# rimelq/VISTAF-RoboSkin-Vision-Integrated-Multimodal-Sensor

Hardware: AMD Instinct MI355X
Metric: frames/sec (224x224 -> force-map) at batch 256 (higher is better)
Workload: dtype f32; 1 GPU; BASELINE configs[2]: batch 256/GPU of 224x224x3 fp16 fringe frames (256 distinct frames) -> 224x224 f32 depth map + force scalars, full FTP path (inpaint, demod, unwrap, detrend, compose, force tail), constants scaled-224; inputs resident in HBM; global_batch=256, input_dtype=fp16, constants=scaled, parallelism=dp1, inflight_batches=3, frames_with_nonzero_status=0

## Files before the change

vistaf-roboskin-vision-integrated-multimodal-sensor_amd/_lib.py:

```python
from __future__ import annotations

import ctypes
import os

_HERE = os.path.dirname(os.path.abspath(__file__))
LIB_PATH = os.path.join(_HERE, "libvistaf_ftp.so")

NSCALARS = 16
NREFINFO = 8
NCONTACT = 16
MAX_CONTACTS = 64
NTRACK = 16
TRACK_NAMES = ["track_id", "age_frames", "parent_row", "events", "overlap_px", "dx", "dy", "dforce_N", "dvolume_cm3", "origin_track_id"]
TRACK_EVENTS = {"born": 1, "split": 2, "merged": 4, "gated": 8}
FATE_ENDED, FATE_NO_ROW = -1, -2 ** 31
NSHAPE = 24
SHAPE_NAMES = ["contact_pixels", "boundary_pixels", "footprint_cx", "footprint_cy", "major_axis_mm", "minor_axis_mm", "orientation_rad",
               "fit_pixels", "fit_status", "apex_x", "apex_y", "apex_depth_mm", "curvature_1_per_mm", "curvature_2_per_mm",
               "curvature_axis_rad", "radius_1_mm", "radius_2_mm", "fit_rms_mm"]
SHAPE_FIT = {"ok": 0, "none": 1, "not_a_cap": 2}
NTAXEL, NTAXELFRAME, TAXEL_NONE = 12, 8, 0xFFFF
TAXEL_NAMES = ["contact_pixels", "contact_area_mm2", "volume_cm3", "mean_depth_mm", "max_depth_mm", "argmax_index", "centroid_x", "centroid_y",
               "force_N", "pressure_kPa"]
TAXEL_FRAME_NAMES = ["active_taxels", "volume_cm3", "force_N", "cop_x", "cop_y", "moment_x_Nmm", "moment_y_Nmm", "peak_taxel"]
# ... 223 lines not shown
        "vistaf_motion_reset": (ci, [vp]),
        "vistaf_motion_destroy": (None, [vp]),
    },
    "PRESSURE_EXPORTS": {
        "vistaf_pressure_create": (ci, [ci, ci, ci, ci, ci, cd, cd, cd, P(vp)]),
        "vistaf_pressure_measure": (ci, [vp, vp, vp, vp, vp, vp, vp, vp, cf, ci, vp, vp, vp, vp]),
        "vistaf_pressure_destroy": (None, [vp]),
    },
}
MASK_CHAIN_SIGNATURES = {
    "vistaf_ftp_test_mask_chain_fits": (ci, [ci, ci, ci, ci, ci, ci]),
    "vistaf_ftp_test_bad_chain": (ci, [vp, vp, vp, vp, vp, ci, ci, vp, vp, ci, ci, ci, ci, vp]),
    "vistaf_ftp_test_reliable_chain": (ci, [vp, vp, vp, ci, ci, ci, vp, vp, vp, vp, ci, ci, ci, ci, vp]),
    "vistaf_ftp_test_contact_chain": (ci, [vp, vp, vp, vp, cd, cd, ci, ci, vp, vp, vp, vp, ci, ci, ci, ci, vp]),
}
OUTLINE_SIGNATURES = {
    "vistaf_outline_workspace_bytes": (ci, [ci, ci, ci, ci, P(sz)]),
    "vistaf_outline_measure": (ci, [vp, vp, vp, vp, ci, ci, ci, ci, ci, vp, vp, vp, vp, sz, vp]),
}
TEXTURE_SIGNATURES = {
    "vistaf_texture_workspace_bytes": (ci, [ci, ci, ci, ci, ci, P(sz)]),
    "vistaf_texture_measure": (ci, [vp, vp, vp, vp, vp, cf, cd, ci, ci, cd, cd, ci, ci, ci, ci, vp, vp, vp, vp, sz, vp]),
}
MATCH_SIGNATURES = {
    "vistaf_match_bank_bytes": (ci, [ci, ci, ci, P(i32), P(sz)]),
    "vistaf_match_build_bank": (ci, [P(cf), P(i32), P(i32), ci, ci, ci, cd, vp, sz]),
    "vistaf_match_workspace_bytes": (ci, [ci, ci, ci, ci, ci, ci, ci, P(sz)]),
    "vistaf_match_measure": (ci, [vp, vp, vp, vp, vp, vp, sz, P(i32), cf, ci, ci, cd, cd, ci, ci, ci, ci, vp, vp, vp, vp, sz, vp]),
}
(EXPORTS, ALIGN_EXPORTS, TEST_EXPORTS, TEMP_EXPORTS, TEMPMODEL_EXPORTS, TSENSOR_EXPORTS, TRACK_EXPORTS, SHAPE_EXPORTS, TAXEL_EXPORTS, THERMAL_EXPORTS,
 TEMPORAL_EXPORTS, CLOUD_EXPORTS, MOTION_EXPORTS, PRESSURE_EXPORTS) = (list(group) for group in SIGNATURES.values())

_lib = None


def load():
    global _lib
    if _lib is not None:
        return _lib
    if not os.path.exists(LIB_PATH):
        raise RuntimeError(
            f"{LIB_PATH} is missing: build it with `python __graft_entry__.py` (hipcc --offload-arch=gfx950). "
            "This package has no CPU path."
        )
    lib = ctypes.CDLL(LIB_PATH)
    for group in list(SIGNATURES.values()) + [MASK_CHAIN_SIGNATURES, OUTLINE_SIGNATURES, TEXTURE_SIGNATURES, MATCH_SIGNATURES]:
        for name, (restype, argtypes) in group.items():
            fn = getattr(lib, name)
            fn.restype, fn.argtypes = restype, argtypes
    _lib = lib
    return lib


def check(rc: int):
    if rc != 0:
        msg = load().vistaf_ftp_last_error().decode("utf-8", "replace")
        if rc == -1:
            raise ValueError(msg)
        raise RuntimeError(f"vistaf_ftp error {rc}: {msg}")
```

vistaf-roboskin-vision-integrated-multimodal-sensor_amd/csrc/api.hip:

```cpp
#include <hip/hip_runtime.h>
#include <algorithm>
#include <cmath>
#include <cstdio>
#include <cstdlib>
#include <cstring>
#include <map>
#include <string>
#include <vector>

#include "host_util.hpp"
#include "mask_rules.hpp"
#include "mask_bits.hpp"

using namespace vf;
#include "test_hooks.h"
#include "test_hooks_masks.h"
#ifdef VISTAF_DEBUG
namespace vf { void telea_debug_dump(); void telea_window_debug_dump(int B); void telea_window_mw_debug_dump(int B); void fit_debug_dump(); void unwrap_big_debug_dump(); void unwrap_batch_debug_dump(); }
#endif

static thread_local std::string g_err;
static int fail(int code, const std::string &msg) { g_err = msg; return code; }
namespace vf { int set_error(int code, const std::string &msg) { return fail(code, msg); } }

namespace {

struct GKern { float *d = nullptr; int k = 0; };

enum Stage { ST_GRAY_BAD = 0, ST_INPAINT, ST_PREPROC, ST_DEMOD, ST_RELIABLE, ST_UNWRAP_RANK, ST_UNWRAP, ST_UNWRAP_TREE, ST_DETREND, ST_SMOOTH_FLIP, ST_COMPOSE, ST_MM_BLOB,
             ST_TAIL, ST_COUNT };
const char *kStageNames[ST_COUNT] = {"gray+badpix", "inpaint (k_telea_window_mw)", "illum+blur+apod+median", "pruned-dft demod", "reliable mask",
// ... 512 lines not shown
    preprocess(hd, d_ref, format, 1, st, false);
    int rc = reference_search(hd, 1, hd->geom, st);
    if (rc) return rc;
    CarrierGeom g;
    HIPCHK(hipMemcpyAsync(&g, hd->geom, sizeof(g), hipMemcpyDeviceToHost, st));
    HIPCHK(hipStreamSynchronize(st));
    if (!g.ok) return fail(VISTAF_E_NOCARRIER, "no carrier peak in the reference spectrum");
    hd->peak_x = g.peak_x; hd->peak_y = g.peak_y; hd->kx = g.kx; hd->ky = g.ky;
    hd->ph = g.ph; hd->pw = g.pw;
    {
        std::vector<float> win = hann_patch(g.ph, g.pw);
        HIPCHK(hipMemcpyAsync(hd->win, win.data(), win.size() * sizeof(float), hipMemcpyHostToDevice, st));
        HIPCHK(hipStreamSynchronize(st));
    }
    launch_build_tables(hd->geom, 0, hd->Ex, hd->Ey, hd->Gx, hd->Gy, 0, 0, 1, h, w, pad, Hf, Wf, hd->pmax, st);
    launch_dft_forward(hd->iw, hd->mu, hd->Ex, hd->Ey, 0, 0, hd->win, hd->tmpT, hd->patch, hd->pmax * hd->pmax, 1, h, w, hd->ph, hd->pw, st);
    launch_dft_inverse(hd->patch, hd->pmax * hd->pmax, hd->Gx, hd->Gy, 0, 0, hd->tmpT, hd->cref, hd->amp_ref, nullptr, nullptr, 0, nullptr, nullptr,
                       1, h, w, hd->ph, hd->pw, st);
    HIPCHK(hipStreamSynchronize(st));
    hd->period = g.period;
    hd->mm_per_px = hd->period > 1e-12 ? c.grating_pitch_mm / hd->period : 0.0;
    hd->have_ref = true;
    return 0;
}

int vistaf_ftp_get_reference_info(const vistaf_ftp_handle *hd, double *o)
{
    if (!hd || !o) return fail(VISTAF_E_INVALID, "null argument");
    if (!hd->have_ref) return fail(VISTAF_E_STATE, "set_reference has not been called");
    o[0] = hd->peak_x; o[1] = hd->peak_y; o[2] = hd->kx; o[3] = hd->ky; o[4] = hd->Hf; o[5] = hd->Wf; o[6] = hd->period; o[7] = hd->mm_per_px;
    return 0;
}

// ... 130 lines not shown
{
    if (!hd || !d_frames) return fail(VISTAF_E_INVALID, "null argument");
    if (!hd->have_ref) return fail(VISTAF_E_STATE, "set_reference has not been called");
    if (B < 1 || B > hd->maxB) return fail(VISTAF_E_STATE, "batch exceeds max_batch");
    TRY(check_frames(hd, format, d_frames, nullptr));
    if (!(hd->period > 1e-12)) return fail(VISTAF_E_STATE, "Invalid estimated_grating_period_px");
    hipStream_t st = (hipStream_t)stream;
    int h = hd->h, w = hd->w;
    bool timed = hd->timing;
    if (timed) ensure_events(hd);
    HIPCHK(hipMemsetAsync(hd->status, 0, sizeof(int32_t) * B, st));

    preprocess(hd, d_frames, format, B, st, timed);

    if (timed) hipEventRecord(hd->ev[ST_DEMOD], st);
    launch_dft_forward(hd->iw, hd->mu, hd->Ex, hd->Ey, 0, 0, hd->win, hd->tmpT, hd->patch, hd->pmax * hd->pmax, B, h, w, hd->ph, hd->pw, st);
    launch_dft_inverse(hd->patch, hd->pmax * hd->pmax, hd->Gx, hd->Gy, 0, 0, hd->tmpT, hd->keep_planes ? hd->field : nullptr, hd->amp, hd->cref,
                       hd->amp_ref, 0, hd->prod, hd->wrapped, B, h, w, hd->ph, hd->pw, st);
    return post_demod(hd, B, d_height_mm, d_reliable, d_scalars, d_status, nullptr, st);
}

int vistaf_ftp_predict_pairs(vistaf_ftp_handle *hd, const void *d_refs, const void *d_defs, int format, int B, float *d_height_mm,
                             uint8_t *d_reliable, double *d_scalars, int32_t *d_status, void *stream)
{
    if (!hd || !d_refs || !d_defs) return fail(VISTAF_E_INVALID, "null argument");
    if (B < 1 || B > hd->maxB) return fail(VISTAF_E_STATE, "batch exceeds max_batch");
    TRY(check_frames(hd, format, d_refs, d_defs));
    hipStream_t st = (hipStream_t)stream;
    const vistaf_ftp_config &c = hd->cfg;
    int h = hd->h, w = hd->w, P = hd->P, pad = std::max(0, c.fft_pad_px), pm = hd->pmax;
    bool timed = hd->timing;
    if (timed) ensure_events(hd);
    if (!hd->pairs_ready) {
// ... 13 lines not shown
    }
    HIPCHK(hipMemsetAsync(hd->status, 0, sizeof(int32_t) * B, st));
    const size_t sx = (size_t)w * pm, sy = (size_t)h * pm;
    const bool together = 2 * B <= hd->maxB;
    const float *iw_def = hd->iw, *mu_def = hd->mu;
    const int *bad_def = hd->bad_count;
    if (together) {
        HIPCHK(hipMemsetAsync(hd->status + B, 0, sizeof(int32_t) * B, st));
        preprocess(hd, d_refs, format, B, st, timed, d_defs);
        iw_def = hd->iw + (size_t)B * P; mu_def = hd->mu + B; bad_def = hd->bad_count + B;
    } else preprocess(hd, d_refs, format, B, st, false);
    int rc = reference_search(hd, B, hd->pgeom, st);
    if (rc) return rc;
    launch_pair_status(hd->pgeom, pm, hd->status, together ? hd->status + B : nullptr, B, st);
    launch_build_tables(hd->pgeom, 1, hd->pEx, hd->pEy, hd->pGx, hd->pGy, sx, sy, B, h, w, pad, hd->Hf, hd->Wf, pm, st, hd->hann_tab, hd->pwin);
    launch_dft_forward(hd->iw, hd->mu, hd->pEx, hd->pEy, sx, sy, hd->pwin, hd->tmpT, hd->patch, pm * pm, B, h, w, pm, pm, st, pm * pm);
    launch_dft_inverse(hd->patch, pm * pm, hd->pGx, hd->pGy, sx, sy, hd->tmpT, hd->pcref, hd->pamp_ref, nullptr, nullptr, 0, nullptr, nullptr, B, h, w,
                       pm, pm, st, hd->pgeom);
    if (!together) preprocess(hd, d_defs, format, B, st, timed);
    if (timed) hipEventRecord(hd->ev[ST_DEMOD], st);
    launch_dft_forward(iw_def, mu_def, hd->pEx, hd->pEy, sx, sy, hd->pwin, hd->tmpT, hd->patch, pm * pm, B, h, w, pm, pm, st, pm * pm);
    launch_dft_inverse(hd->patch, pm * pm, hd->pGx, hd->pGy, sx, sy, hd->tmpT, hd->keep_planes ? hd->field : nullptr, hd->amp, hd->pcref, hd->pamp_ref,
                       (size_t)P, hd->prod, hd->wrapped, B, h, w, pm, pm, st, hd->pgeom);
    return post_demod(hd, B, d_height_mm, d_reliable, d_scalars, d_status, hd->pgeom, st, bad_def);
}

int vistaf_ftp_get_pair_info(vistaf_ftp_handle *hd, int batch, double *out , void *stream)
{
    if (!hd || !out) return fail(VISTAF_E_INVALID, "null argument");
    if (!hd->pairs_ready || batch < 1 || batch > hd->maxB) return fail(VISTAF_E_STATE, "predict_pairs has not been called");
    std::vector<CarrierGeom> g(batch);
    HIPCHK(hipMemcpyAsync(g.data(), hd->pgeom, sizeof(CarrierGeom) * batch, hipMemcpyDeviceToHost, (hipStream_t)stream));
    HIPCHK(hipStreamSynchronize((hipStream_t)stream));
    for (int b = 0; b < batch; b++) {
        double *o = out + (size_t)b * VISTAF_NREFINFO;
        o[0] = g[b].peak_x; o[1] = g[b].peak_y; o[2] = g[b].kx; o[3] = g[b].ky; o[4] = hd->Hf; o[5] = hd->Wf; o[6] = g[b].period;
        o[7] = g[b].period > 1e-12 ? hd->cfg.grating_pitch_mm / g[b].period : 0.0;
    }
// ... 41 lines not shown
int vistaf_ftp_test_set(vistaf_ftp_handle *hd, const char *name, int value)
{
    if (!hd || !name) return fail(VISTAF_E_INVALID, "null argument");
    const std::string n(name);
    if (n == "inpaint_tier" && value >= 0 && value <= 2) hd->tiers.inpaint = value;
    else if (n == "big_flood_handback") hd->tiers.big_flood_handback = value != 0;
    else if (n == "chamfer_twopass") hd->tiers.chamfer_twopass = value != 0;
    else if (n == "telea_two_tier") hd->tiers.telea_two_tier = value != 0;
    else if (n == "telea_mw") hd->tiers.telea_mw = value != 0;
    else if (n == "big_queue_lds") hd->tiers.big_queue_lds = value != 0;
    else if (n == "big_gq_cap" && (value == 0 || (value >= 64 && (value & (value - 1)) == 0))) hd->tiers.big_gq_cap = value;
    else if (n == "big_fallback") hd->tiers.big_fallback = value != 0;
    else if (n == "unwrap_fast") hd->tiers.unwrap_fast = value != 0;
    else if (n == "big_chain") hd->tiers.big_chain = value != 0;
    else if (n == "select_resident") hd->tiers.select_resident = value != 0;
    else if (n == "fused_chains") hd->tiers.fused_chains = value != 0;
    else if (n == "fused_backend") hd->tiers.fused_backend = value != 0;
    else if (n == "fused_masks" && value >= 0 && value <= 7) hd->tiers.fused_masks = value;
    else if (n == "keep_planes") hd->keep_planes = value != 0;
    else return fail(VISTAF_E_INVALID, "unknown test hook or value: " + n);
    return 0;
}

namespace {
int hook_scratch(int variant, int B, int h, int w, bool chain_ok, void **scratch)
{
    *scratch = nullptr;
    if (variant < 0 || variant > 2) return fail(VISTAF_E_INVALID, "variant must be 0, 1 or 2");
    if (variant == 2 && !chain_ok) return fail(VISTAF_E_INVALID, "variant 2: the k_big.hip chain does not take this batch");
    if (variant == 1 || (variant == 0 && !large_frame((size_t)h * w))) return 0;
// ... 405 lines not shown
        (void)hipFree(geom); (void)hipFree(hann);
        return fail(VISTAF_E_HIP, "memcpy geometry");
    }
    launch_build_tables(geom, geom_stride, (double2 *)Ex, (double2 *)Ey, (double2 *)Gx, (double2 *)Gy, (size_t)w * pmax, (size_t)h * pmax, B, h, w, pad, Hf,
                        Wf, pmax, st, pair ? hann : nullptr, pair ? win : nullptr);
    return hook_finish(geom, hann, st);
}

int vistaf_ftp_test_build_full_tables(void *Exf, void *Eyf, int h, int w, int pad, int Hf, int Wf, void *stream)
{
    if (!Exf || !Eyf || !dft_sizes_ok(1, h, w) || !padded_ok(h, w, pad, Hf, Wf)) return fail(VISTAF_E_INVALID, "bad argument");
    launch_build_full_tables((double2 *)Exf, (double2 *)Eyf, h, w, pad, Hf, Wf, (hipStream_t)stream);
    return hook_finish(nullptr, nullptr, (hipStream_t)stream);
}

int vistaf_ftp_test_dft_forward(const float *iw, const float *mu, const void *Ex, const void *Ey, size_t tab_stride_x, size_t tab_stride_y, const float *win,
                                int win_stride, void *T, void *patch, int patch_stride, int B, int h, int w, int ph, int pw, void *stream)
{
    if (!iw || !Ex || !Ey || !win || !T || !patch || !dft_sizes_ok(B, h, w) || ph < 1 || pw < 1 || ph > 4096 || pw > 4096 ||
        (size_t)B * h * pw > 0x7fffffffull)
        return fail(VISTAF_E_INVALID, "bad argument");
    if ((tab_stride_x == 0) != (tab_stride_y == 0) || (tab_stride_x && (tab_stride_x < (size_t)w * pw || tab_stride_y < (size_t)ph * h)) ||
        (win_stride != 0 && win_stride < ph * pw) || patch_stride < ph * pw)
        return fail(VISTAF_E_INVALID, "a stride is smaller than what it strides over, or only one table stride is zero");
    launch_dft_forward(iw, mu, (const double2 *)Ex, (const double2 *)Ey, tab_stride_x, tab_stride_y, win, (double2 *)T, (double2 *)patch, patch_stride, B, h, w,
                       ph, pw, (hipStream_t)stream, win_stride);
    return hook_finish(nullptr, nullptr, (hipStream_t)stream);
}

int vistaf_ftp_test_dft_inverse(const void *patch, int patch_stride, const void *Gx, const void *Gy, size_t tab_stride_x, size_t tab_stride_y, void *Q, void *field,
                                float *amp, const void *cref, const float *amp_ref, size_t ref_stride, float *prod, float *wrapped, const int32_t *gi_or_null,
                                int B, int h, int w, int ph, int pw, void *stream)
{
    if (!patch || !Gx || !Gy || !Q || !amp || (cref && (!amp_ref || !prod || !wrapped)) || !dft_sizes_ok(B, h, w) || ph < 1 || pw < 1 || ph > 4096 ||
        pw > 4096 || (size_t)B * ph * w > 0x7fffffffull)
        return fail(VISTAF_E_INVALID, "bad argument");
    if ((tab_stride_x == 0) != (tab_stride_y == 0) || (tab_stride_x && (tab_stride_x < (size_t)w * pw || tab_stride_y < (size_t)ph * h)) ||
        patch_stride < ph * pw || (ref_stride != 0 && ref_stride < (size_t)h * w))
        return fail(VISTAF_E_INVALID, "a stride is smaller than what it strides over, or only one table stride is zero");
    hipStream_t st = (hipStream_t)stream;
    CarrierGeom *geom = nullptr;
    if (gi_or_null) {
        const double zeros[7] = {0, 0, 0, 0, 0, 0, 0};
        std::vector<CarrierGeom> g((size_t)B);
        for (int b = 0; b < B; b++) g[b] = geom_pack(zeros, gi_or_null + 10 * (size_t)b);
        HIPCHK(hipMalloc((void **)&geom, g.size() * sizeof(CarrierGeom)));
        if (hipMemcpy(geom, g.data(), g.size() * sizeof(CarrierGeom), hipMemcpyHostToDevice) != hipSuccess) {
            (void)hipFree(geom);
            return fail(VISTAF_E_HIP, "memcpy geometry");
        }
    }
    launch_dft_inverse((const double2 *)patch, patch_stride, (const double2 *)Gx, (const double2 *)Gy, tab_stride_x, tab_stride_y, (double2 *)Q, (double2 *)field, amp,
                       (const double2 *)cref, amp_ref, ref_stride, prod, wrapped, B, h, w, ph, pw, st, geom);
    return hook_finish(geom, nullptr, st);
}

int vistaf_depth_map_to_volume(const float *d_height, const uint8_t *d_roi, int batch, int h, int w, double mm_per_px,
                               double depth_eps_mm, double *d_out, void *stream)
{
    if (!d_height || !d_out || batch < 1 || h < 1 || w < 1) return fail(VISTAF_E_INVALID, "bad argument");
    PostParams pp;
    pp.mm_per_px = mm_per_px; pp.depth_eps_mm = depth_eps_mm; pp.period_px = 0; pp.force_curve = Curve{0, 0, 0, 0};
    launch_tail(d_height, d_roi, nullptr, nullptr, pp, nullptr, 0, d_out, batch, h * w, (hipStream_t)stream);
    return launch_ok("launch");
}

int vistaf_predict_force_from_volume(const vistaf_curve *curve, double volume_cm3, double *force_out)
{
// ... 9 lines not shown
```

vistaf-roboskin-vision-integrated-multimodal-sensor_amd/csrc/cgemm_mfma.hpp:

```cpp
#pragma once
#include <hip/hip_runtime.h>

namespace vf {

typedef double v4f64 __attribute__((ext_vector_type(4)));

__device__ __forceinline__ void cgemm16x64_mfma(const double *__restrict__ A, int lda, int kext, const double2 *__restrict__ Q, int ldq, int ncols,
                                                int ya, int x0, int lane, v4f64 (&cre)[4], v4f64 (&cim)[4])
{
    const int r = lane & 15, kk = lane >> 4;
#pragma unroll
    for (int t = 0; t < 4; t++) { cre[t] = (v4f64){0.0, 0.0, 0.0, 0.0}; cim[t] = (v4f64){0.0, 0.0, 0.0, 0.0}; }
    const int K = 2 * kext;
    for (int k0 = 0; k0 < K; k0 += 4) {
        const int k = k0 + kk;
        const bool in = k < K, hi = k >= kext;
        const int kq = in ? (hi ? k - kext : k) : 0;
        const double a = in ? A[((size_t)ya * lda + kq) * 2 + (hi ? 1 : 0)] : 0.0;
        double2 q[4];
#pragma unroll
        for (int t = 0; t < 4; t++) q[t] = Q[(size_t)kq * ldq + min(x0 + 16 * t + r, ncols - 1)];
#pragma unroll
        for (int t = 0; t < 4; t++) {
            const double bre = in ? (hi ? -q[t].y : q[t].x) : 0.0, bim = in ? (hi ? q[t].x : q[t].y) : 0.0;
            cre[t] = __builtin_amdgcn_mfma_f64_16x16x4f64(a, bre, cre[t], 0, 0, 0);
            cim[t] = __builtin_amdgcn_mfma_f64_16x16x4f64(a, bim, cim[t], 0, 0, 0);
        }
    }
}

}
```

vistaf-roboskin-vision-integrated-multimodal-sensor_amd/csrc/k_dft.hip:

```cpp
#include <algorithm>
#include "kernels.hpp"
#include "cgemm_mfma.hpp"

namespace vf {

__device__ inline void cmac(double &ar, double &ai, double er, double ei, double vr, double vi)
{
    ar = fma(er, vr, ar); ar = fma(-ei, vi, ar);
    ai = fma(er, vi, ai); ai = fma(ei, vr, ai);
}

constexpr int DFT_MAXT = 4;
__global__ __launch_bounds__(256) void k_dft_fwd1_mfma(const float *__restrict__ iw, const float *__restrict__ mu, const double2 *__restrict__ Ex_all,
                                                       size_t ex_stride, double2 *__restrict__ T, int h, int w, int pw, int seg_rows, int nseg)
{
    const int lane = threadIdx.x & 63, wid = threadIdx.x >> 6;
    const int sps = (seg_rows + 15) / 16;
    const int strip = blockIdx.x * 4 + wid;
    if (strip >= nseg * sps) return;
    const int seg = strip / sps;
    const int row0 = seg * seg_rows + (strip - seg * sps) * 16;
    const int row_end = (seg + 1) * seg_rows;
    const int r = lane & 15, kk = lane >> 4;
    const int grow = min(row0 + r, row_end - 1);
// ... 22 lines not shown
                if (t0 + t < ntile) acc[t] = __builtin_amdgcn_mfma_f64_16x16x4f64(a, bv[t], acc[t], 0, 0, 0);
        }
#pragma unroll
        for (int t = 0; t < DFT_MAXT; t++) {
            if (eoff[t] < 0) continue;
            const int n = (t0 + t) * 16 + r, c = n < pw ? n : n - pw;
#pragma unroll
            for (int q = 0; q < 4; q++) {
                const int row = row0 + kk + 4 * q;
                if (row < row_end) ((double *)(T + (size_t)row * pw + c))[n < pw ? 0 : 1] = acc[t][q];
            }
        }
    }
}

__global__ void k_dft_fwd2(const double2 *__restrict__ T, const double2 *__restrict__ Ey_all, size_t ey_stride, const float *__restrict__ win_all,
                           int win_stride, double2 *__restrict__ patch, int h, int ph, int pw, int pstride)
{
    size_t b = blockIdx.x;
    const double2 *Ey = Ey_all + b * ey_stride;
    const float *win = win_all + b * (size_t)win_stride;
    const double2 *Tb = T + b * (size_t)h * pw;
    for (int t = threadIdx.x; t < ph * pw; t += blockDim.x) {
        int a = t / pw, c = t % pw;
        double ar = 0.0, ai = 0.0;
        int y = 0;
        for (; y + 8 <= h; y += 8) {
            double2 e[8], v[8];
#pragma unroll
            for (int k = 0; k < 8; k++) { e[k] = Ey[(size_t)a * h + y + k]; v[k] = Tb[(size_t)(y + k) * pw + c]; }
#pragma unroll
            for (int k = 0; k < 8; k++) cmac(ar, ai, e[k].x, e[k].y, v[k].x, v[k].y);
        }
        for (; y < h; y++) {
            const double2 e = Ey[(size_t)a * h + y], v = Tb[(size_t)y * pw + c];
            cmac(ar, ai, e.x, e.y, v.x, v.y);
        }
        const double wv = (double)win[t];
        patch[b * (size_t)pstride + t] = make_double2(ar * wv, ai * wv);
    }
}

void launch_dft_forward(const float *iw, const float *mu, const double2 *Ex, const double2 *Ey, size_t tab_stride_x, size_t tab_stride_y,
                        const float *win, double2 *tmpT, double2 *patch, int patch_stride, int B, int h, int w, int ph, int pw, hipStream_t st,
                        int win_stride)
{
    const int seg_rows = tab_stride_x ? h : B * h, nseg = tab_stride_x ? B : 1;
    const int strips = nseg * ((seg_rows + 15) / 16);
    hipLaunchKernelGGL(k_dft_fwd1_mfma, dim3((strips + 3) / 4), dim3(256), 0, st, iw, mu, Ex, tab_stride_x, tmpT, h, w, pw, seg_rows, nseg);
    hipLaunchKernelGGL(k_dft_fwd2, dim3(B), dim3(std::min(1024, ((ph * pw + 63) / 64) * 64)), 0, st, (const double2 *)tmpT, Ey, tab_stride_y, win, win_stride, patch, h,
                       ph, pw, patch_stride);
}

__global__ void k_dft_inv1(const double2 *__restrict__ patch, int pstride, const double2 *__restrict__ Gx_all, size_t gx_stride,
                           double2 *__restrict__ Q, int w, int ph, int pw, const CarrierGeom *__restrict__ geom)
{
    int x = blockIdx.x * blockDim.x + threadIdx.x;
    int a = blockIdx.y;
    size_t b = blockIdx.z;
    if (x >= w) return;
    const int pwb = geom ? max(0, min(geom[b].pw, pw)) : pw;
    if (geom && a >= max(0, min(geom[b].ph, ph))) return;
    const double2 *Gx = Gx_all + b * gx_stride;
    const double2 *pr = patch + b * (size_t)pstride + (size_t)a * pw;
// ... 35 lines not shown
            const size_t p = (size_t)y * w + x, i = b * (size_t)h * w + p;
            if (field) field[i] = make_double2(ar, ai);
            const float am = (float)sqrt(fma(ar, ar, ai * ai));
            amp[i] = am;
            if (cref) {
                const double2 c = cref[p];
                const double rr = ar * c.x + ai * c.y;
                const double ri = ai * c.x - ar * c.y;
                wrapped[i] = (float)atan2(ri, rr);
                prod[i] = __fmul_rn(amp_ref[p], am);
            }
        }
    }
}

void launch_dft_inverse(const double2 *patch, int patch_stride, const double2 *Gx, const double2 *Gy, size_t tab_stride_x, size_t tab_stride_y,
                        double2 *tmpQ, double2 *field, float *amp, const double2 *cref, const float *amp_ref, size_t ref_stride, float *prod,
                        float *wrapped, int B, int h, int w, int ph, int pw, hipStream_t st, const CarrierGeom *geom)
{
    hipLaunchKernelGGL(k_dft_inv1, dim3((w + 255) / 256, ph, B), dim3(256), 0, st, patch, patch_stride, Gx, tab_stride_x, tmpQ, w, ph, pw, geom);
    hipLaunchKernelGGL(k_dft_inv2_mfma, dim3((w + 63) / 64, (h + 63) / 64, B), dim3(256), 0, st, (const double2 *)tmpQ, Gy, tab_stride_y, field, amp, cref,
                       amp_ref, ref_stride, prod, wrapped, h, w, ph, geom);
}

__global__ __launch_bounds__(256) void k_full2_mfma(const double2 *__restrict__ T, const double2 *__restrict__ Eyf, double *__restrict__ mag_all,
                                                    int h, int Hf, int Wf, int Wh)
{
    const int lane = threadIdx.x & 63, wid = threadIdx.x >> 6;
    const int x0 = blockIdx.x * 64, y0 = (blockIdx.y * 4 + wid) * 16;
    const size_t b = blockIdx.z;
    if (y0 >= Hf) return;
    const int r = lane & 15, kk = lane >> 4;
    const double *G = (const double *)Eyf;
    const double2 *Tb = T + b * (size_t)h * Wh;
    const int ya = min(y0 + r, Hf - 1);
    v4f64 cre[4], cim[4];
    cgemm16x64_mfma(G, h, h, Tb, Wh, Wh, ya, x0, lane, cre, cim);
// ... 147 lines not shown
```

vistaf-roboskin-vision-integrated-multimodal-sensor_amd/csrc/kernels.hpp:

```cpp
#pragma once
#include <hip/hip_runtime.h>
#include <stdint.h>
#include <vector>
#include "common.hpp"

namespace vf {

struct Tiers {
    int inpaint = 2;
    int big_flood_handback = 0;
    int chamfer_twopass = 0;
    int telea_two_tier = 1;
    int unwrap_fast = 1;
    int big_chain = 1;
    int big_queue_lds = 1;
    int big_gq_cap = 0;
    int big_fallback = 1;
    int telea_mw = 1;
    int fused_backend = 1;
    int select_resident = 1;
    int fused_masks = 7;
    int fused_chains = 1;
};

inline bool large_frame(size_t P) { return P >= 262144; }

struct ScratchLayout;
struct ScratchRegion;
using ScratchRec = std::vector<ScratchRegion>;

struct RowSpanSE {
    int k;
    int8_t lo[33];
    int8_t hi[33];
};

// ... 35 lines not shown
                          float *const *outs, int *counts, int B, int P, hipStream_t st);

struct CarrierGeom {
    double peak_x, peak_y;
    double kx, ky;
    double dpx, dpy;
    double period;
    int x0, y0, ph, pw;
    int px_i, py_i;
    int px_raw, py_raw;
    int ok;
    int keep_carrier;
};
void launch_dft_forward(const float *iw, const float *mu, const double2 *Ex, const double2 *Ey, size_t tab_stride_x, size_t tab_stride_y,
                        const float *win, double2 *tmpT, double2 *patch, int patch_stride, int B, int h, int w, int ph, int pw, hipStream_t st,
                        int win_stride = 0);
void launch_dft_inverse(const double2 *patch, int patch_stride, const double2 *Gx, const double2 *Gy, size_t tab_stride_x, size_t tab_stride_y,
                        double2 *tmpQ, double2 *field, float *amp, const double2 *cref, const float *amp_ref, size_t ref_stride, float *prod,
                        float *wrapped, int B, int h, int w, int ph, int pw, hipStream_t st, const CarrierGeom *geom = nullptr);
void launch_dft_full_mag(const float *iw, const float *mu, const double2 *Ex_full, const double2 *Ey_full, double2 *tmp,
                         double *mag, int B, int h, int w, int Hf, int Wf, hipStream_t st);
void launch_dft_rows(const float *iw, const float *mu, const double2 *Ex, double2 *T, int B, int h, int w, int nc, hipStream_t st);
void launch_top_peaks(const double *mag, int B, int Hf, int Wf, int dc, int npeaks, double *out_xyv , hipStream_t st);
void launch_carrier_choose(const double *peaks, int npk, const double *mag, int Hf, int Wf, int bw, double max_dy_frac, CarrierGeom *geom, int B,
                           hipStream_t st);
void launch_build_tables(const CarrierGeom *geom, int geom_stride, double2 *Ex, double2 *Ey, double2 *Gx, double2 *Gy, size_t stride_x,
                         size_t stride_y, int B, int h, int w, int pad, int Hf, int Wf, int pmax, hipStream_t st, const float *pair_hann = nullptr,
                         float *pair_win = nullptr);
void launch_pair_status(const CarrierGeom *geom, int pmax, int32_t *status, const int32_t *status2, int B, hipStream_t st);
void launch_build_full_tables(double2 *Exf, double2 *Eyf, int h, int w, int pad, int Hf, int Wf, hipStream_t st);

void launch_threshold_mask(const float *q, const uint8_t *roi, const float *thr, uint8_t *out, int B, int P, hipStream_t st);
enum CcLabelTier { CCT_LDS_MASK = 0, CCT_LDS = 1, CCT_GLOBAL = 2 };
int cc_label_tier(int h, int w, bool force_global = false);
// ... 161 lines not shown
```

Before: 75890 frames/s.

## Add LDS-staged MFMA kernels for forward row DFT and inverse column DFT

Measured after the change: 76690 frames/s, median of 6. 1.01x the previous value.

```diff
diff --git a/vistaf-roboskin-vision-integrated-multimodal-sensor_amd/_lib.py b/vistaf-roboskin-vision-integrated-multimodal-sensor_amd/_lib.py
--- a/vistaf-roboskin-vision-integrated-multimodal-sensor_amd/_lib.py
+++ b/vistaf-roboskin-vision-integrated-multimodal-sensor_amd/_lib.py
@@ -261,6 +261,11 @@
     "vistaf_ftp_test_reliable_chain": (ci, [vp, vp, vp, ci, ci, ci, vp, vp, vp, vp, ci, ci, ci, ci, vp]),
     "vistaf_ftp_test_contact_chain": (ci, [vp, vp, vp, vp, cd, cd, ci, ci, vp, vp, vp, vp, ci, ci, ci, ci, vp]),
 }
+DFT_STAGED_SIGNATURES = {
+    "vistaf_ftp_test_dft_forward_v": (ci, [vp, vp, vp, vp, sz, sz, vp, ci, vp, vp, ci, ci, ci, ci, ci, ci, ci, vp]),
+    "vistaf_ftp_test_dft_inverse_v": (ci, [vp, ci, vp, vp, sz, sz, vp, vp, vp, vp, vp, sz, vp, vp, vp, ci, ci, ci, ci, ci, ci, vp]),
+    "vistaf_ftp_test_dft_staged_fits": (ci, [ci, ci, ci, ci, ci]),
+}
 OUTLINE_SIGNATURES = {
     "vistaf_outline_workspace_bytes": (ci, [ci, ci, ci, ci, P(sz)]),
     "vistaf_outline_measure": (ci, [vp, vp, vp, vp, ci, ci, ci, ci, ci, vp, vp, vp, vp, sz, vp]),
@@ -291,7 +296,7 @@
             "This package has no CPU path."
         )
     lib = ctypes.CDLL(LIB_PATH)
-    for group in list(SIGNATURES.values()) + [MASK_CHAIN_SIGNATURES, OUTLINE_SIGNATURES, TEXTURE_SIGNATURES, MATCH_SIGNATURES]:
+    for group in list(SIGNATURES.values()) + [MASK_CHAIN_SIGNATURES, DFT_STAGED_SIGNATURES, OUTLINE_SIGNATURES, TEXTURE_SIGNATURES, MATCH_SIGNATURES]:
         for name, (restype, argtypes) in group.items():
             fn = getattr(lib, name)
             fn.restype, fn.argtypes = restype, argtypes
diff --git a/vistaf-roboskin-vision-integrated-multimodal-sensor_amd/csrc/api.hip b/vistaf-roboskin-vision-integrated-multimodal-sensor_amd/csrc/api.hip
--- a/vistaf-roboskin-vision-integrated-multimodal-sensor_amd/csrc/api.hip
+++ b/vistaf-roboskin-vision-integrated-multimodal-sensor_amd/csrc/api.hip
@@ -15,6 +15,7 @@
 using namespace vf;
 #include "test_hooks.h"
 #include "test_hooks_masks.h"
+#include "test_hooks_dft.h"
 #ifdef VISTAF_DEBUG
 namespace vf { void telea_debug_dump(); void telea_window_debug_dump(int B); void telea_window_mw_debug_dump(int B); void fit_debug_dump(); void unwrap_big_debug_dump(); void unwrap_batch_debug_dump(); }
 #endif
@@ -557,9 +558,9 @@
         HIPCHK(hipStreamSynchronize(st));
     }
     launch_build_tables(hd->geom, 0, hd->Ex, hd->Ey, hd->Gx, hd->Gy, 0, 0, 1, h, w, pad, Hf, Wf, hd->pmax, st);
-    launch_dft_forward(hd->iw, hd->mu, hd->Ex, hd->Ey, 0, 0, hd->win, hd->tmpT, hd->patch, hd->pmax * hd->pmax, 1, h, w, hd->ph, hd->pw, st);
+    launch_dft_forward(hd->iw, hd->mu, hd->Ex, hd->Ey, 0, 0, hd->win, hd->tmpT, hd->patch, hd->pmax * hd->pmax, 1, h, w, hd->ph, hd->pw, st, 0, hd->tiers.dft_staged != 0);
     launch_dft_inverse(hd->patch, hd->pmax * hd->pmax, hd->Gx, hd->Gy, 0, 0, hd->tmpT, hd->cref, hd->amp_ref, nullptr, nullptr, 0, nullptr, nullptr,
-                       1, h, w, hd->ph, hd->pw, st);
+                       1, h, w, hd->ph, hd->pw, st, nullptr, hd->tiers.dft_staged != 0);
     HIPCHK(hipStreamSynchronize(st));
     hd->period = g.period;
     hd->mm_per_px = hd->period > 1e-12 ? c.grating_pitch_mm / hd->period : 0.0;
@@ -720,9 +721,9 @@
     preprocess(hd, d_frames, format, B, st, timed);
 
     if (timed) hipEventRecord(hd->ev[ST_DEMOD], st);
-    launch_dft_forward(hd->iw, hd->mu, hd->Ex, hd->Ey, 0, 0, hd->win, hd->tmpT, hd->patch, hd->pmax * hd->pmax, B, h, w, hd->ph, hd->pw, st);
+    launch_dft_forward(hd->iw, hd->mu, hd->Ex, hd->Ey, 0, 0, hd->win, hd->tmpT, hd->patch, hd->pmax * hd->pmax, B, h, w, hd->ph, hd->pw, st, 0, hd->tiers.dft_staged != 0);
     launch_dft_inverse(hd->patch, hd->pmax * hd->pmax, hd->Gx, hd->Gy, 0, 0, hd->tmpT, hd->keep_planes ? hd->field : nullptr, hd->amp, hd->cref,
-                       hd->amp_ref, 0, hd->prod, hd->wrapped, B, h, w, hd->ph, hd->pw, st);
+                       hd->amp_ref, 0, hd->prod, hd->wrapped, B, h, w, hd->ph, hd->pw, st, nullptr, hd->tiers.dft_staged != 0);
     return post_demod(hd, B, d_height_mm, d_reliable, d_scalars, d_status, nullptr, st);
 }
 
@@ -766,14 +767,14 @@
     if (rc) return rc;
     launch_pair_status(hd->pgeom, pm, hd->status, together ? hd->status + B : nullptr, B, st);
     launch_build_tables(hd->pgeom, 1, hd->pEx, hd->pEy, hd->pGx, hd->pGy, sx, sy, B, h, w, pad, hd->Hf, hd->Wf, pm, st, hd->hann_tab, hd->pwin);
-    launch_dft_forward(hd->iw, hd->mu, hd->pEx, hd->pEy, sx, sy, hd->pwin, hd->tmpT, hd->patch, pm * pm, B, h, w, pm, pm, st, pm * pm);
+    launch_dft_forward(hd->iw, hd->mu, hd->pEx, hd->pEy, sx, sy, hd->pwin, hd->tmpT, hd->patch, pm * pm, B, h, w, pm, pm, st, pm * pm, hd->tiers.dft_staged != 0);
     launch_dft_inverse(hd->patch, pm * pm, hd->pGx, hd->pGy, sx, sy, hd->tmpT, hd->pcref, hd->pamp_ref, nullptr, nullptr, 0, nullptr, nullptr, B, h, w,
-                       pm, pm, st, hd->pgeom);
+                       pm, pm, st, hd->pgeom, hd->tiers.dft_staged != 0);
     if (!together) preprocess(hd, d_defs, format, B, st, timed);
     if (timed) hipEventRecord(hd->ev[ST_DEMOD], st);
-    launch_dft_forward(iw_def, mu_def, hd->pEx, hd->pEy, sx, sy, hd->pwin, hd->tmpT, hd->patch, pm * pm, B, h, w, pm, pm, st, pm * pm);
+    launch_dft_forward(iw_def, mu_def, hd->pEx, hd->pEy, sx, sy, hd->pwin, hd->tmpT, hd->patch, pm * pm, B, h, w, pm, pm, st, pm * pm, hd->tiers.dft_staged != 0);
     launch_dft_inverse(hd->patch, pm * pm, hd->pGx, hd->pGy, sx, sy, hd->tmpT, hd->keep_planes ? hd->field : nullptr, hd->amp, hd->pcref, hd->pamp_ref,
-                       (size_t)P, hd->prod, hd->wrapped, B, h, w, pm, pm, st, hd->pgeom);
+                       (size_t)P, hd->prod, hd->wrapped, B, h, w, pm, pm, st, hd->pgeom, hd->tiers.dft_staged != 0);
     return post_demod(hd, B, d_height_mm, d_reliable, d_scalars, d_status, hd->pgeom, st, bad_def);
 }
 
@@ -845,6 +846,7 @@
     else if (n == "unwrap_fast") hd->tiers.unwrap_fast = value != 0;
     else if (n == "big_chain") hd->tiers.big_chain = value != 0;
     else if (n == "select_resident") hd->tiers.select_resident = value != 0;
+    else if (n == "dft_staged") hd->tiers.dft_staged = value != 0;
     else if (n == "fused_chains") hd->tiers.fused_chains = value != 0;
     else if (n == "fused_backend") hd->tiers.fused_backend = value != 0;
     else if (n == "fused_masks" && value >= 0 && value <= 7) hd->tiers.fused_masks = value;
@@ -1280,8 +1282,24 @@
     return hook_finish(nullptr, nullptr, (hipStream_t)stream);
 }
 
+namespace {
+int dft_hook_variant(int variant, int bit, int h, int w, int ph, int pw, bool per_frame, bool *staged)
+{
+    if (variant < 0 || variant > 2) return fail(VISTAF_E_INVALID, "variant must be 0, 1 or 2");
+    if (variant == 2 && !(dft_staged_fits(h, w, ph, pw, per_frame) & bit)) return fail(VISTAF_E_INVALID, "variant 2: the staged kernel does not take this shape");
+    *staged = variant != 1;
+    return 0;
+}
+}
+
 int vistaf_ftp_test_dft_forward(const float *iw, const float *mu, const void *Ex, const void *Ey, size_t tab_stride_x, size_t tab_stride_y, const float *win,
                                 int win_stride, void *T, void *patch, int patch_stride, int B, int h, int w, int ph, int pw, void *stream)
+{
+    return vistaf_ftp_test_dft_forward_v(iw, mu, Ex, Ey, tab_stride_x, tab_stride_y, win, win_stride, T, patch, patch_stride, B, h, w, ph, pw, 0, stream);
+}
+
+int vistaf_ftp_test_dft_forward_v(const float *iw, const float *mu, const void *Ex, const void *Ey, size_t tab_stride_x, size_t tab_stride_y, const float *win,
+                                  int win_stride, void *T, void *patch, int patch_stride, int B, int h, int w, int ph, int pw, int variant, void *stream)
 {
     if (!iw || !Ex || !Ey || !win || !T || !patch || !dft_sizes_ok(B, h, w) || ph < 1 || pw < 1 || ph > 4096 || pw > 4096 ||
         (size_t)B * h * pw > 0x7fffffffull)
@@ -1289,8 +1307,10 @@
     if ((tab_stride_x == 0) != (tab_stride_y == 0) || (tab_stride_x && (tab_stride_x < (size_t)w * pw || tab_stride_y < (size_t)ph * h)) ||
         (win_stride != 0 && win_stride < ph * pw) || patch_stride < ph * pw)
         return fail(VISTAF_E_INVALID, "a stride is smaller than what it strides over, or only one table stride is zero");
+    bool staged;
+    if (int rc = dft_hook_variant(variant, DFT_STAGED_FWD1, h, w, ph, pw, tab_stride_x != 0, &staged)) return rc;
     launch_dft_forward(iw, mu, (const double2 *)Ex, (const double2 *)Ey, tab_stride_x, tab_stride_y, win, (double2 *)T, (double2 *)patch, patch_stride, B, h, w,
-                       ph, pw, (hipStream_t)stream, win_stride);
+                       ph, pw, (hipStream_t)stream, win_stride, staged);
     return hook_finish(nullptr, nullptr, (hipStream_t)stream);
 }
 
@@ -1298,12 +1318,28 @@
                                 float *amp, const void *cref, const float *amp_ref, size_t ref_stride, float *prod, float *wrapped, const int32_t *gi_or_null,
                                 int B, int h, int w, int ph, int pw, void *stream)
 {
+    return vistaf_ftp_test_dft_inverse_v(patch, patch_stride, Gx, Gy, tab_stride_x, tab_stride_y, Q, field, amp, cref, amp_ref, ref_stride, prod, wrapped,
+                                         gi_or_null, B, h, w, ph, pw, 0, stream);
+}
+
+int vistaf_ftp_test_dft_staged_fits(int h, int w, int ph, int pw, int per_frame_tables)
+{
+    if (h < 1 || w < 1 || ph < 1 || pw < 1) return fail(VISTAF_E_INVALID, "bad argument");
+    return dft_staged_fits(h, w, ph, pw, per_frame_tables != 0);
+}
+
+int vistaf_ftp_test_dft_inverse_v(const void *patch, int patch_stride, const void *Gx, const void *Gy, size_t tab_stride_x, size_t tab_stride_y, void *Q,
+                                  void *field, float *amp, const void *cref, const float *amp_ref, size_t ref_stride, float *prod, float *wrapped,
+                                  const int32_t *gi_or_null, int B, int h, int w, int ph, int pw, int variant, void *stream)
+{
     if (!patch || !Gx || !Gy || !Q || !amp || (cref && (!amp_ref || !prod || !wrapped)) || !dft_sizes_ok(B, h, w) || ph < 1 || pw < 1 || ph > 4096 ||
         pw > 4096 || (size_t)B * ph * w > 0x7fffffffull)
         return fail(VISTAF_E_INVALID, "bad argument");
     if ((tab_stride_x == 0) != (tab_stride_y == 0) || (tab_stride_x && (tab_stride_x < (size_t)w * pw || tab_stride_y < (size_t)ph * h)) ||
         patch_stride < ph * pw || (ref_stride != 0 && ref_stride < (size_t)h * w))
         return fail(VISTAF_E_INVALID, "a stride is smaller than what it strides over, or only one table stride is zero");
+    bool staged;
+    if (int rc = dft_hook_variant(variant, DFT_STAGED_INV2, h, w, ph, pw, tab_stride_x != 0, &staged)) return rc;
     hipStream_t st = (hipStream_t)stream;
     CarrierGeom *geom = nullptr;
     if (gi_or_null) {
@@ -1317,7 +1353,7 @@
         }
     }
     launch_dft_inverse((const double2 *)patch, patch_stride, (const double2 *)Gx, (const double2 *)Gy, tab_stride_x, tab_stride_y, (double2 *)Q, (double2 *)field, amp,
-                       (const double2 *)cref, amp_ref, ref_stride, prod, wrapped, B, h, w, ph, pw, st, geom);
+                       (const double2 *)cref, amp_ref, ref_stride, prod, wrapped, B, h, w, ph, pw, st, geom, staged);
     return hook_finish(geom, nullptr, st);
 }
 
diff --git a/vistaf-roboskin-vision-integrated-multimodal-sensor_amd/csrc/cgemm_mfma.hpp b/vistaf-roboskin-vision-integrated-multimodal-sensor_amd/csrc/cgemm_mfma.hpp
--- a/vistaf-roboskin-vision-integrated-multimodal-sensor_amd/csrc/cgemm_mfma.hpp
+++ b/vistaf-roboskin-vision-integrated-multimodal-sensor_amd/csrc/cgemm_mfma.hpp
@@ -29,4 +29,30 @@
     }
 }
 
+template <int NT>
+__device__ __forceinline__ void cgemm16_lds_mfma(const double *sA, int lda, int kext, const double2 *sQ, int ra, int t0, int lane, v4f64 (&cre)[NT],
+                                                 v4f64 (&cim)[NT])
+{
+    const int r = lane & 15, kk = lane >> 4;
+#pragma unroll
+    for (int t = 0; t < NT; t++) { cre[t] = (v4f64){0.0, 0.0, 0.0, 0.0}; cim[t] = (v4f64){0.0, 0.0, 0.0, 0.0}; }
+    const int K = 2 * kext;
+    for (int k0 = 0; k0 < K; k0 += 4) {
+        const int k = k0 + kk;
+        const bool in = k < K, hi = k >= kext;
+        const int kq = in ? (hi ? k - kext : k) : 0;
+        const double av = sA[(ra * lda + kq) * 2 + (hi ? 1 : 0)];
+        const double a = in ? av : 0.0;
+        double2 q[NT];
+#pragma unroll
+        for (int t = 0; t < NT; t++) q[t] = sQ[kq * 64 + 16 * (t0 + t) + r];
+#pragma unroll
+        for (int t = 0; t < NT; t++) {
+            const double bre = in ? (hi ? -q[t].y : q[t].x) : 0.0, bim = in ? (hi ? q[t].x : q[t].y) : 0.0;
+            cre[t] = __builtin_amdgcn_mfma_f64_16x16x4f64(a, bre, cre[t], 0, 0, 0);
+            cim[t] = __builtin_amdgcn_mfma_f64_16x16x4f64(a, bim, cim[t], 0, 0, 0);
+        }
+    }
 }
+
+}
diff --git a/vistaf-roboskin-vision-integrated-multimodal-sensor_amd/csrc/k_dft.hip b/vistaf-roboskin-vision-integrated-multimodal-sensor_amd/csrc/k_dft.hip
--- a/vistaf-roboskin-vision-integrated-multimodal-sensor_amd/csrc/k_dft.hip
+++ b/vistaf-roboskin-vision-integrated-multimodal-sensor_amd/csrc/k_dft.hip
@@ -60,6 +60,112 @@
     }
 }
 
+constexpr int FWD1_MAXPW = 24;
+constexpr int INV2_MAXPH = 22;
+int dft_staged_fits(int h, int w, int ph, int pw, bool per_frame_tables)
+{
+    (void)per_frame_tables;
+    if (h < 1 || w < 1 || ph < 1 || pw < 1) return 0;
+    return (pw <= FWD1_MAXPW ? DFT_STAGED_FWD1 : 0) | (ph <= INV2_MAXPH ? DFT_STAGED_INV2 : 0);
+}
+
+constexpr int FWD1_XC = 32, FWD1_EST = 48, FWD1_IST = 36;
+constexpr int FWD1_NLE = FWD1_XC * FWD1_MAXPW / 256, FWD1_NLI = 16 * FWD1_XC / 64;
+constexpr int FWD1_LDS_E = FWD1_XC * FWD1_EST * 8, FWD1_LDS_I = 16 * FWD1_IST * 4, FWD1_LDS_O = 16 * FWD1_MAXPW * 16;
+constexpr int FWD1_LDS = FWD1_LDS_E + 4 * FWD1_LDS_I > 4 * FWD1_LDS_O ? FWD1_LDS_E + 4 * FWD1_LDS_I : 4 * FWD1_LDS_O;
+template <int NT>
+__global__ __launch_bounds__(256, 4) void k_dft_fwd1_staged(const float *__restrict__ iw, const float *__restrict__ mu, const double2 *__restrict__ Ex_all,
+                                                         size_t ex_stride, double2 *__restrict__ T, int h, int w, int pw, int seg_rows, int nseg)
+{
+    __shared__ __attribute__((aligned(16))) unsigned char s_raw[FWD1_LDS];
+    double *sE = (double *)s_raw;
+    const int lane = threadIdx.x & 63, wid = threadIdx.x >> 6;
+    float *sI = (float *)(s_raw + FWD1_LDS_E) + wid * (16 * FWD1_IST);
+    const int sps = (seg_rows + 15) / 16, wgps = (sps + 3) / 4;
+    const int seg = blockIdx.x / wgps, sstrip = (blockIdx.x - seg * wgps) * 4 + wid;
+    const bool active = sstrip < sps;
+    const int row0 = seg * seg_rows + sstrip * 16;
+    const int row_end = (seg + 1) * seg_rows;
+    const int r = lane & 15, kk = lane >> 4;
+    const int grow = active ? min(row0 + r, row_end - 1) : 0;
+    const double2 *E = Ex_all + (size_t)seg * ex_stride;
+    const float m = (mu && active) ? mu[grow / h] : 0.f;
+    const int ncol = 2 * pw;
+    v4f64 acc[NT];
+    bool colv[NT];
+#pragma unroll
+    for (int t = 0; t < NT; t++) {
+        acc[t] = (v4f64){0.0, 0.0, 0.0, 0.0};
+        colv[t] = t * 16 + r < ncol;
+    }
+    double2 ve[FWD1_NLE];
+    float vi[FWD1_NLI];
+    auto fetch = [&](int xc0) {
+        const int ne = min(FWD1_XC, w - xc0) * pw;
+#pragma unroll
+        for (int j = 0; j < FWD1_NLE; j++) ve[j] = E[(size_t)xc0 * pw + min((int)threadIdx.x + 256 * j, ne - 1)];
+        if (active) {
+#pragma unroll
+            for (int j = 0; j < FWD1_NLI; j++) {
+                const int e = lane + 64 * j, rr = e / FWD1_XC, x = xc0 + e % FWD1_XC;
+                vi[j] = iw[(size_t)min(row0 + rr, row_end - 1) * w + min(x, w - 1)];
+            }
+        }
+    };
+    fetch(0);
+    for (int xc0 = 0; xc0 < w; xc0 += FWD1_XC) {
+        if (xc0) __syncthreads();
+        const int ne = min(FWD1_XC, w - xc0) * pw;
+#pragma unroll
+        for (int j = 0; j < FWD1_NLE; j++) {
+            const int e = threadIdx.x + 256 * j;
+            if (e < ne) {
+                const int xl = e / pw, c = e - xl * pw;
+                sE[xl * FWD1_EST + c] = ve[j].x;
+                sE[xl * FWD1_EST + pw + c] = ve[j].y;
+            }
+        }
+        if (active) {
+#pragma unroll
+            for (int j = 0; j < FWD1_NLI; j++) {
+                const int e = lane + 64 * j, rr = e / FWD1_XC, xl = e % FWD1_XC;
+                sI[rr * FWD1_IST + xl] = xc0 + xl < w ? vi[j] : 0.f;
+            }
+        }
+        __syncthreads();
+        if (xc0 + FWD1_XC < w) fetch(xc0 + FWD1_XC);
+        if (active) {
+            const int nk = min(FWD1_XC, w - xc0);
+            for (int xl = 0; xl < nk; xl += 4) {
+                const bool in = xc0 + xl + kk < w;
+                const float af = sI[r * FWD1_IST + xl + kk];
+                const double a = in ? (double)__fsub_rn(af, m) : 0.0;
+                double bv[NT];
+#pragma unroll
+                for (int t = 0; t < NT; t++) bv[t] = sE[(xl + kk) * FWD1_EST + t * 16 + r];
+#pragma unroll
+                for (int t = 0; t < NT; t++) acc[t] = __builtin_amdgcn_mfma_f64_16x16x4f64(a, (in && colv[t]) ? bv[t] : 0.0, acc[t], 0, 0, 0);
+            }
+        }
+    }
+    __syncthreads();
+    double2 *sO = (double2 *)s_raw + wid * (16 * FWD1_MAXPW);
+    if (active) {
+#pragma unroll
+        for (int t = 0; t < NT; t++) {
+            if (!colv[t]) continue;
+            const int n = t * 16 + r, c = n < pw ? n : n - pw;
+#pragma unroll
+            for (int q = 0; q < 4; q++) ((double *)(sO + (kk + 4 * q) * pw + c))[n < pw ? 0 : 1] = acc[t][q];
+        }
+    }
+    __syncthreads();
+    if (active) {
+        const int no = min(16, row_end - row0) * pw;
+        for (int e = lane; e < no; e += 64) T[(size_t)row0 * pw + e] = sO[e];
+    }
+}
+
 __global__ void k_dft_fwd2(const double2 *__restrict__ T, const double2 *__restrict__ Ey_all, size_t ey_stride, const float *__restrict__ win_all,
                            int win_stride, double2 *__restrict__ patch, int h, int ph, int pw, int pstride)
 {
@@ -89,11 +195,17 @@
 
 void launch_dft_forward(const float *iw, const float *mu, const double2 *Ex, const double2 *Ey, size_t tab_stride_x, size_t tab_stride_y,
                         const float *win, double2 *tmpT, double2 *patch, int patch_stride, int B, int h, int w, int ph, int pw, hipStream_t st,
-                        int win_stride)
+                        int win_stride, bool staged)
 {
     const int seg_rows = tab_stride_x ? h : B * h, nseg = tab_stride_x ? B : 1;
-    const int strips = nseg * ((seg_rows + 15) / 16);
-    hipLaunchKernelGGL(k_dft_fwd1_mfma, dim3((strips + 3) / 4), dim3(256), 0, st, iw, mu, Ex, tab_stride_x, tmpT, h, w, pw, seg_rows, nseg);
+    const int sps = (seg_rows + 15) / 16, strips = nseg * sps;
+    if (staged && (dft_staged_fits(h, w, ph, pw, tab_stride_x != 0) & DFT_STAGED_FWD1)) {
+        const dim3 grid(nseg * ((sps + 3) / 4));
+        if (pw <= 8) hipLaunchKernelGGL(k_dft_fwd1_staged<1>, grid, dim3(256), 0, st, iw, mu, Ex, tab_stride_x, tmpT, h, w, pw, seg_rows, nseg);
+        else if (pw <= 16) hipLaunchKernelGGL(k_dft_fwd1_staged<2>, grid, dim3(256), 0, st, iw, mu, Ex, tab_stride_x, tmpT, h, w, pw, seg_rows, nseg);
+        else hipLaunchKernelGGL(k_dft_fwd1_staged<3>, grid, dim3(256), 0, st, iw, mu, Ex, tab_stride_x, tmpT, h, w, pw, seg_rows, nseg);
+    } else
+        hipLaunchKernelGGL(k_dft_fwd1_mfma, dim3((strips + 3) / 4), dim3(256), 0, st, iw, mu, Ex, tab_stride_x, tmpT, h, w, pw, seg_rows, nseg);
     hipLaunchKernelGGL(k_dft_fwd2, dim3(B), dim3(std::min(1024, ((ph * pw + 63) / 64) * 64)), 0, st, (const double2 *)tmpT, Ey, tab_stride_y, win, win_stride, patch, h,
                        ph, pw, patch_stride);
 }
@@ -159,13 +271,100 @@
     }
 }
 
+__device__ __forceinline__ void inv2_finish_tile(const v4f64 &cre, const v4f64 &cim, int x, int y, size_t b, int h, int w, double2 *__restrict__ field,
+                                                 float *__restrict__ amp, bool cref, const double2 (&cv)[4], const float (&av)[4],
+                                                 float *__restrict__ prod, float *__restrict__ wrapped)
+{
+    if (x >= w) return;
+#pragma unroll
+    for (int qd = 0; qd < 4; qd++, y += 4) {
+        if (y >= h) continue;
+        const double ar = cre[qd], ai = cim[qd];
+        const size_t p = (size_t)y * w + x, i = b * (size_t)h * w + p;
+        if (field) field[i] = make_double2(ar, ai);
+        const float am = (float)sqrt(fma(ar, ar, ai * ai));
+        amp[i] = am;
+        if (cref) {
+            const double2 c = cv[qd];
+            const double rr = ar * c.x + ai * c.y;
+            const double ri = ai * c.x - ar * c.y;
+            wrapped[i] = (float)atan2(ri, rr);
+            prod[i] = __fmul_rn(av[qd], am);
+        }
+    }
+}
+
+constexpr int INV2_NT = 2;
+__global__ __launch_bounds__(256, 3) void k_dft_inv2_staged(const double2 *__restrict__ Q, const double2 *__restrict__ Gy_all, size_t gy_stride,
+                                                         double2 *__restrict__ field, float *__restrict__ amp, const double2 *__restrict__ cref_all,
+                                                         const float *__restrict__ amp_ref_all, size_t ref_stride, float *__restrict__ prod,
+                                                         float *__restrict__ wrapped, int h, int w, int ph, const CarrierGeom *__restrict__ geom)
+{
+    extern __shared__ double2 s_inv2[];
+    const int lane = threadIdx.x & 63, wid = threadIdx.x >> 6;
+    const int x0 = blockIdx.x * 64, y0 = (blockIdx.y * 4 + wid) * 16;
+    const size_t b = blockIdx.z;
+    const int r = lane & 15, kk = lane >> 4;
+    const double2 *Qb = Q + b * (size_t)ph * w;
+    const int phb = geom ? max(0, min(geom[b].ph, ph)) : ph;
+    double2 *sQ = s_inv2, *sG = s_inv2 + ph * 64 + wid * 16 * ph;
+    constexpr int NLD = (INV2_MAXPH * 64 + 255) / 256;
+    const int spare = ph * 128 + threadIdx.x;
+    if (phb > 0) {
+        double2 v[NLD];
+        const int c = min(x0 + lane, w - 1);
+#pragma unroll
+        for (int j = 0; j < NLD; j++) v[j] = Qb[(size_t)min(wid + 4 * j, phb - 1) * w + c];
+#pragma unroll
+        for (int j = 0; j < NLD; j++) sQ[wid + 4 * j < phb ? (wid + 4 * j) * 64 + lane : spare] = v[j];
+    }
+    if (y0 < h) {
+        const double2 *Gs = Gy_all + b * gy_stride + (size_t)y0 * ph;
+        const int n = min(16, h - y0) * ph;
+        double2 v[NLD];
+#pragma unroll
+        for (int j = 0; j < NLD; j++) v[j] = Gs[min(lane + 64 * j, n - 1)];
+#pragma unroll
+        for (int j = 0; j < NLD; j++) (lane + 64 * j < n ? sG + lane + 64 * j : sQ + spare)[0] = v[j];
+    }
+    __syncthreads();
+    if (y0 >= h) return;
+    const int ra = min(r, h - 1 - y0);
+    const double2 *cref = cref_all ? cref_all + b * ref_stride : nullptr;
+    const float *amp_ref = amp_ref_all ? amp_ref_all + b * ref_stride : nullptr;
+    for (int t0 = 0; t0 < 4 && x0 + 16 * t0 < w; t0 += INV2_NT) {
+        v4f64 cre[INV2_NT], cim[INV2_NT];
+        double2 cv[INV2_NT][4];
+        float av[INV2_NT][4];
+        if (cref) {
+#pragma unroll
+            for (int t = 0; t < INV2_NT; t++)
+#pragma unroll
+                for (int qd = 0; qd < 4; qd++) {
+                    const size_t p = (size_t)min(y0 + kk + 4 * qd, h - 1) * w + min(x0 + 16 * (t0 + t) + r, w - 1);
+                    cv[t][qd] = cref[p];
+                    av[t][qd] = amp_ref[p];
+                }
+        }
+        cgemm16_lds_mfma<INV2_NT>((const double *)sG, ph, phb, sQ, ra, t0, lane, cre, cim);
+#pragma unroll
+        for (int t = 0; t < INV2_NT; t++)
+            inv2_finish_tile(cre[t], cim[t], x0 + 16 * (t0 + t) + r, y0 + kk, b, h, w, field, amp, cref != nullptr, cv[t], av[t], prod, wrapped);
+    }
+}
+
 void launch_dft_inverse(const double2 *patch, int patch_stride, const double2 *Gx, const double2 *Gy, size_t tab_stride_x, size_t tab_stride_y,
                         double2 *tmpQ, double2 *field, float *amp, const double2 *cref, const float *amp_ref, size_t ref_stride, float *prod,
-                        float *wrapped, int B, int h, int w, int ph, int pw, hipStream_t st, const CarrierGeom *geom)
+                        float *wrapped, int B, int h, int w, int ph, int pw, hipStream_t st, const CarrierGeom *geom, bool staged)
 {
     hipLaunchKernelGGL(k_dft_inv1, dim3((w + 255) / 256, ph, B), dim3(256), 0, st, patch, patch_stride, Gx, tab_stride_x, tmpQ, w, ph, pw, geom);
-    hipLaunchKernelGGL(k_dft_inv2_mfma, dim3((w + 63) / 64, (h + 63) / 64, B), dim3(256), 0, st, (const double2 *)tmpQ, Gy, tab_stride_y, field, amp, cref,
-                       amp_ref, ref_stride, prod, wrapped, h, w, ph, geom);
+    const dim3 grid((w + 63) / 64, (h + 63) / 64, B);
+    if (staged && (dft_staged_fits(h, w, ph, pw, tab_stride_x != 0) & DFT_STAGED_INV2))
+        hipLaunchKernelGGL(k_dft_inv2_staged, grid, dim3(256), (size_t)ph * 2048 + 4096, st, (const double2 *)tmpQ, Gy, tab_stride_y, field, amp, cref, amp_ref,
+                           ref_stride, prod, wrapped, h, w, ph, geom);
+    else
+        hipLaunchKernelGGL(k_dft_inv2_mfma, grid, dim3(256), 0, st, (const double2 *)tmpQ, Gy, tab_stride_y, field, amp, cref, amp_ref, ref_stride, prod,
+                           wrapped, h, w, ph, geom);
 }
 
 __global__ __launch_bounds__(256) void k_full2_mfma(const double2 *__restrict__ T, const double2 *__restrict__ Eyf, double *__restrict__ mag_all,
diff --git a/vistaf-roboskin-vision-integrated-multimodal-sensor_amd/csrc/kernels.hpp b/vistaf-roboskin-vision-integrated-multimodal-sensor_amd/csrc/kernels.hpp
--- a/vistaf-roboskin-vision-integrated-multimodal-sensor_amd/csrc/kernels.hpp
+++ b/vistaf-roboskin-vision-integrated-multimodal-sensor_amd/csrc/kernels.hpp
@@ -20,6 +20,7 @@
     int fused_backend = 1;
     int select_resident = 1;
     int fused_masks = 7;
+    int dft_staged = 1;
     int fused_chains = 1;
 };
 
@@ -85,10 +86,12 @@
 };
 void launch_dft_forward(const float *iw, const float *mu, const double2 *Ex, const double2 *Ey, size_t tab_stride_x, size_t tab_stride_y,
                         const float *win, double2 *tmpT, double2 *patch, int patch_stride, int B, int h, int w, int ph, int pw, hipStream_t st,
-                        int win_stride = 0);
+                        int win_stride = 0, bool staged = true);
 void launch_dft_inverse(const double2 *patch, int patch_stride, const double2 *Gx, const double2 *Gy, size_t tab_stride_x, size_t tab_stride_y,
                         double2 *tmpQ, double2 *field, float *amp, const double2 *cref, const float *amp_ref, size_t ref_stride, float *prod,
-                        float *wrapped, int B, int h, int w, int ph, int pw, hipStream_t st, const CarrierGeom *geom = nullptr);
+                        float *wrapped, int B, int h, int w, int ph, int pw, hipStream_t st, const CarrierGeom *geom = nullptr, bool staged = true);
+enum DftStaged { DFT_STAGED_FWD1 = 1, DFT_STAGED_INV2 = 2 };
+int dft_staged_fits(int h, int w, int ph, int pw, bool per_frame_tables);
 void launch_dft_full_mag(const float *iw, const float *mu, const double2 *Ex_full, const double2 *Ey_full, double2 *tmp,
                          double *mag, int B, int h, int w, int Hf, int Wf, hipStream_t st);
 void launch_dft_rows(const float *iw, const float *mu, const double2 *Ex, double2 *T, int B, int h, int w, int nc, hipStream_t st);
```
